# adaly/gridnext

Measured on AMD Instinct MI355X. Metric: spots/sec training throughput (multimodal f+g), higher is better.
Workload: dtype f32; 1 GPU; C4: multimodal f(DenseNet-121 @128px + count-MLP 2000 genes) + hex g on 78x64 Visium grids, 1 array (4992 spots) per GPU per step, f frozen/eval (tutorial mode), g trained with Adam, masked CE; spots_per_array=4992, parallelism=dp1

## Files before the change

### gridnext_amd/csrc/conv3x3.hip

```cpp
#include "fwd_common.h"

namespace {

constexpr int C3_BM = 128, C3_BN = 32;

__global__ __launch_bounds__(256) void conv3x3_kernel(const float* __restrict__ A, long lda,
                                                      const float* __restrict__ Wr, float* __restrict__ out, long ldc,
                                                      long M, int N, int K, int S, const float* __restrict__ scale,
                                                      const float* __restrict__ shift, int vecA, int vecW) {
    extern __shared__ __attribute__((aligned(16))) float lds[];
    const int strip = C3_BM + 2 * S + 2;
    float* As = lds;
    float* Bs = lds + strip * LDK;
    const int t = threadIdx.x, lane = t & 63, wave = t >> 6, h = lane >> 5, i = lane & 31;
    const long P0 = (long)blockIdx.x * C3_BM;
    const long base = P0 - S - 1;
    const int n0 = blockIdx.y * C3_BN;
    const bool has_act = scale != nullptr;

    const long P = P0 + 32 * wave + i;
    unsigned mask = 0;
    if (P < M) {
        const int rem = (int)(P % ((long)S * S));
        const int y = rem / S, x = rem - y * S;
#pragma unroll
        for (int tap = 0; tap < 9; ++tap) {
            const int yy = y + tap / 3 - 1, xx = x + tap % 3 - 1;
            if (yy >= 0 && yy < S && xx >= 0 && xx < S) mask |= 1u << tap;
        }
    }
    f32x16 acc;
#pragma unroll
    for (int r = 0; r < 16; ++r) acc[r] = 0.f;

    const int kq = t & 7;
    for (int k0 = 0; k0 < K; k0 += 32) {
        const int k = k0 + 4 * kq;
        const int valid = K - k;
        float4 sc4 = make_float4(1.f, 1.f, 1.f, 1.f), sh4 = make_float4(0.f, 0.f, 0.f, 0.f);
        if (has_act && valid > 0) {
            sc4 = ld4_safe(scale + k, valid, vecA);
            sh4 = ld4_safe(shift + k, valid, vecA);
        }
        __syncthreads();
        for (int row = t >> 3; row < strip; row += 32) {
            const long Pr = base + row;
            float4 v = make_float4(0.f, 0.f, 0.f, 0.f);
            if (Pr >= 0 && Pr < M && valid > 0) {
                v = ld4_safe(A + Pr * lda + k, valid, vecA);
                if (has_act) v = act4(v, sc4, sh4);
                if (valid < 4) {
                    if (valid < 2) v.y = 0.f;
                    if (valid < 3) v.z = 0.f;
                    v.w = 0.f;
                }
            }
            *reinterpret_cast<float4*>(&As[row * LDK + 4 * kq]) = v;
        }
        for (int idx = t >> 3; idx < 9 * 32; idx += 32) {
            const int tap = idx >> 5, n = n0 + (idx & 31);
            float4 v = make_float4(0.f, 0.f, 0.f, 0.f);
            if (n < N && valid > 0) v = ld4_safe(Wr + ((long)tap * N + n) * K + k, valid, vecW);
            *reinterpret_cast<float4*>(&Bs[idx * LDK + 4 * kq]) = v;
        }
        __syncthreads();
#pragma unroll
        for (int tap = 0; tap < 9; ++tap) {
            const int off = (S + 1) + (tap / 3 - 1) * S + (tap % 3 - 1);
            const bool ok = (mask >> tap) & 1u;
            const float* ap = &As[(32 * wave + i + off) * LDK + 4 * h];
            const float* bp = &Bs[(tap * 32 + i) * LDK + 4 * h];
#pragma unroll
            for (int s = 0; s < 4; ++s) {
                float4 a = ld4(ap + 8 * s);
                const float4 b = ld4(bp + 8 * s);
                if (!ok) a = make_float4(0.f, 0.f, 0.f, 0.f);
                acc = __builtin_amdgcn_mfma_f32_32x32x2f32(a.x, b.x, acc, 0, 0, 0);
                acc = __builtin_amdgcn_mfma_f32_32x32x2f32(a.y, b.y, acc, 0, 0, 0);
                acc = __builtin_amdgcn_mfma_f32_32x32x2f32(a.z, b.z, acc, 0, 0, 0);
                acc = __builtin_amdgcn_mfma_f32_32x32x2f32(a.w, b.w, acc, 0, 0, 0);
            }
        }
    }
    const int col = n0 + i;
    if (col < N) {
#pragma unroll
        for (int r = 0; r < 16; ++r) {
            const long row = P0 + 32 * wave + (r & 3) + 8 * (r >> 2) + 4 * h;
            if (row < M) out[row * ldc + col] = acc[r];
        }
    }
}

template <int NJ>
__global__ __launch_bounds__(256) void conv3x3_pipe_kernel(const float* __restrict__ A, long lda,
                                                           const float* __restrict__ Wr, float* __restrict__ out,
                                                           long ldc, long M, int N, int K, int S,
                                                           const float* __restrict__ scale,
                                                           const float* __restrict__ shift, int vecA, int vecW) {
    extern __shared__ __attribute__((aligned(16))) float lds[];
    const int strip = C3_BM + 2 * S + 2;
    float* As = lds;
    float* Bs = lds + strip * LDK;
    const int t = threadIdx.x, lane = t & 63, wave = t >> 6, h = lane >> 5, i = lane & 31;
    const long P0 = (long)blockIdx.x * C3_BM;
    const long base = P0 - S - 1;
    const int n0 = blockIdx.y * C3_BN;
    const bool has_act = scale != nullptr;
    const int kq = t & 7, r0 = t >> 3;

    const long P = P0 + 32 * wave + i;
    unsigned mask = 0;
    if (P < M) {
        const int rem = (int)(P % ((long)S * S));
        const int y = rem / S, x = rem - y * S;
#pragma unroll
        for (int tap = 0; tap < 9; ++tap) {
            const int yy = y + tap / 3 - 1, xx = x + tap % 3 - 1;
            if (yy >= 0 && yy < S && xx >= 0 && xx < S) mask |= 1u << tap;
        }
    }
    f32x16 acc0, acc1;
#pragma unroll
    for (int r = 0; r < 16; ++r) { acc0[r] = 0.f; acc1[r] = 0.f; }
    float* Zs = Bs + 9 * 32 * LDK;
    if (t < LDK) Zs[t] = 0.f;
    int aoff[9];
#pragma unroll
    for (int tap = 0; tap < 9; ++tap) {
        const int off = (S + 1) + (tap / 3 - 1) * S + (tap % 3 - 1);
        aoff[tap] = ((mask >> tap) & 1u) ? (32 * wave + i + off) * LDK + 4 * h : (strip + 9 * 32) * LDK;
    }

    float4 ra[NJ], rb[9], sc4, sh4;
    const int nload = n0 + r0 < N ? n0 + r0 : N - 1;
    auto fetch = [&](int k0) {
        const int k = k0 + 4 * kq;
        const int kc = k < K ? k : 0;
        sc4 = make_float4(1.f, 1.f, 1.f, 1.f);
        sh4 = make_float4(0.f, 0.f, 0.f, 0.f);
        if (has_act) {
            sc4 = ld4(scale + kc);
            sh4 = ld4(shift + kc);
        }
#pragma unroll
        for (int j = 0; j < NJ; ++j) {
            long Pr = base + r0 + 32 * j;
            Pr = Pr < 0 ? 0 : (Pr >= M ? M - 1 : Pr);
            ra[j] = ld4(A + Pr * lda + kc);
        }
#pragma unroll
        for (int j = 0; j < 9; ++j) rb[j] = ld4(Wr + ((long)j * N + nload) * K + kc);
    };
    const bool interior = base >= 0 && base + strip <= M && (K & 31) == 0 && n0 + C3_BN <= N;
    auto stash = [&](int k0) {
        if (interior) {
#pragma unroll
            for (int j = 0; j < NJ; ++j) {
                const int row = r0 + 32 * j;
                if (row >= strip) continue;
                float4 v = ra[j];
                if (has_act) v = act4(v, sc4, sh4);
                *reinterpret_cast<float4*>(&As[row * LDK + 4 * kq]) = v;
            }
#pragma unroll
            for (int j = 0; j < 9; ++j) *reinterpret_cast<float4*>(&Bs[(r0 + 32 * j) * LDK + 4 * kq]) = rb[j];
            return;
        }
        const bool kok = k0 + 4 * kq < K;
        const bool nok = n0 + r0 < N;
#pragma unroll
        for (int j = 0; j < NJ; ++j) {
            const int row = r0 + 32 * j;
            if (row >= strip) continue;
            const long Pr = base + row;
            float4 v = ra[j];
            if (has_act) v = act4(v, sc4, sh4);
            if (!(kok && Pr >= 0 && Pr < M)) v = make_float4(0.f, 0.f, 0.f, 0.f);
            *reinterpret_cast<float4*>(&As[row * LDK + 4 * kq]) = v;
        }
#pragma unroll
        for (int j = 0; j < 9; ++j) {
            float4 v = rb[j];
            if (!(kok && nok)) v = make_float4(0.f, 0.f, 0.f, 0.f);
            *reinterpret_cast<float4*>(&Bs[(r0 + 32 * j) * LDK + 4 * kq]) = v;
        }
    };

    const float* bbase = &Bs[i * LDK + 4 * h];
    fetch(0);
    __syncthreads();
    stash(0);
    __syncthreads();
    for (int k0 = 0; k0 < K; k0 += 32) {
        __builtin_amdgcn_s_setprio(3);
        if (k0 + 32 < K) fetch(k0 + 32);
        __builtin_amdgcn_s_setprio(0);
        float4 a = ld4(lds + aoff[0]), b = ld4(bbase);
#pragma unroll
        for (int step = 0; step < 36; ++step) {
            const int tap = step >> 2, sidx = step & 3;
            float4 na = a, nb = b;
            if (step < 35) {
                const int ntap = (step + 1) >> 2, ns = (step + 1) & 3;
                na = ld4(lds + aoff[ntap] + 8 * ns);
                nb = ld4(bbase + ntap * 32 * LDK + 8 * ns);
            }
            (void)tap; (void)sidx;
            acc0 = __builtin_amdgcn_mfma_f32_32x32x2f32(a.x, b.x, acc0, 0, 0, 0);
            acc1 = __builtin_amdgcn_mfma_f32_32x32x2f32(a.y, b.y, acc1, 0, 0, 0);
            acc0 = __builtin_amdgcn_mfma_f32_32x32x2f32(a.z, b.z, acc0, 0, 0, 0);
            acc1 = __builtin_amdgcn_mfma_f32_32x32x2f32(a.w, b.w, acc1, 0, 0, 0);
            a = na; b = nb;
            __builtin_amdgcn_sched_group_barrier(0x100, 2, 0);
            __builtin_amdgcn_sched_group_barrier(0x008, 4, 0);
        }
        if (k0 + 32 < K) {
            __builtin_amdgcn_s_setprio(3);
            __syncthreads();
            stash(k0 + 32);
            __syncthreads();
            __builtin_amdgcn_s_setprio(0);
        }
    }
    __builtin_amdgcn_s_setprio(3);
    const int col = n0 + i;
    if (col < N) {
#pragma unroll
        for (int r = 0; r < 16; ++r) {
            const long row = P0 + 32 * wave + (r & 3) + 8 * (r >> 2) + 4 * h;
            if (row < M) out[row * ldc + col] = acc0[r] + acc1[r];
        }
    }
}

#ifndef GNX_DMA_DBG
#define GNX_DMA_DBG 0
#endif

struct C3BnAdj {
    const float* a; int lda;
    const float* sc; const float* sh; const float* mean; const float* inv;
    float* slab;
};
template <int S, int NW, int KC, bool NK1 = false, bool H16 = false, bool O16 = false, bool BNADJ = false>
__global__ __launch_bounds__(64 * NW) void conv3x3_dma_kernel(const float* __restrict__ A, int lda,
                                                              const float* __restrict__ Wr, float* __restrict__ out,
                                                              int ldc, int M, int K, int N, C3BnAdj bn = C3BnAdj()) {
    constexpr int BM = 32 * NW;
    constexpr int strip = BM + 2 * S + 2;
    constexpr int SR = (strip + 15) & ~15;
    constexpr int ROWB = KC * 4;
    constexpr int GB = 16 * ROWB, PPG = GB / 1024;
    constexpr int BUFB = (SR + 9 * 32) * ROWB;
    constexpr int NPA = (SR >> 4) * PPG, NPW = 18 * PPG;
    constexpr int NSA = (NPA + NW - 1) / NW, NSW = (NPW + NW - 1) / NW;
    constexpr int SPT = KC / 8, STEPS = 9 * SPT;
    constexpr int ZB = 2 * BUFB;
    static_assert(NSA + NSW <= STEPS, "one DMA slot per MFMA step");
    static_assert(ZB + 2048 <= 160 * 1024, "LDS");
    __shared__ __attribute__((aligned(16))) char lds[ZB + 2048];
    const int t = threadIdx.x, lane = t & 63, h = lane >> 5, i = lane & 31;
    const int wave = __builtin_amdgcn_readfirstlane(t >> 6);
    for (int z = t; z < 512; z += 64 * NW) reinterpret_cast<float*>(lds + ZB)[z] = 0.f;
    const int T = M / BM;
    const int nk2 = NK1 ? N / 64 : K / (2 * KC);
    int G = gridDim.x;
    asm volatile("" : "+s"(G));
#ifndef GNX_XCD_ORDER
#define GNX_XCD_ORDER 1
#endif
    const int bx = blockIdx.x;
#if GNX_XCD_ORDER == 2
    const int bid = (G & 31) == 0 ? ((bx >> 5) << 5) + ((bx & 7) << 2) + ((bx >> 3) & 3) : bx;
#else
    const int bid = (GNX_XCD_ORDER && (G & 7) == 0) ? (bx & 7) * (G >> 3) + (bx >> 3) : bx;
#endif
    auto tile_of = [&](int round) {
        const int base = round * G;
        return base + (base + G <= T ? bid : bx);
    };
    const unsigned lb = lds_addr(lds);

    const unsigned voffA = ((unsigned)(lane & 15) * lda + 4 * (lane >> 4)) * 4u;
    const unsigned voffW = ((unsigned)(lane & 15) * K + 4 * (lane >> 4)) * 4u;
    int nround = 0, ntile = tile_of(0), nchunk = 0;
    const __amdgpu_buffer_rsrc_t rW = __builtin_amdgcn_make_buffer_rsrc(const_cast<float*>(Wr), 0, 9 * N * K * 4, 0x00020000);
    auto issue_slot = [&](auto slot_c, char* dst) {
        constexpr int slot = decltype(slot_c)::value;
        if constexpr (slot < NSA) {
            const int p = wave + NW * slot;
            if ((NPA % NW) && slot == NSA - 1 && p >= NPA) return;
            const int grp = p / PPG, part = p % PPG;
            const int row0 = ntile * BM - S - 1 + 16 * grp;
            char* d = dst + grp * GB + part * 1024;
            if (__builtin_expect(row0 >= 0 && row0 + 15 < M, 1)) {
                const __amdgpu_buffer_rsrc_t rs = __builtin_amdgcn_make_buffer_rsrc(
                    const_cast<float*>(A + (long)row0 * lda), 0, (15 * lda + K) * 4, 0x00020000);
                dma16_buf(rs, voffA, ((NK1 ? 0 : KC * nchunk) + 16 * part) * 4, lds_addr(d));
            } else {
                int Pr = row0 + (lane & 15);
                Pr = Pr < 0 ? 0 : (Pr >= M ? M - 1 : Pr);
                dma16_global(A + (long)Pr * lda + (NK1 ? 0 : KC * nchunk) + 16 * part + 4 * (lane >> 4), lds_addr(d));
            }
        } else {
            const int p = wave + NW * (slot - NSA);
            if ((NPW % NW) && slot == NSA + NSW - 1 && p >= NPW) return;
            if (H16 && !NK1 && nk2 == 1 && nround > 0) return;
            const int grp = p / PPG, part = p % PPG;
            dma16_buf(rW, voffW,
                      (((grp >> 1) * N + (NK1 ? 32 * nchunk : 0) + (grp & 1) * 16) * K + (NK1 ? 0 : KC * nchunk) + 16 * part) * 4,
                      lds_addr(dst + SR * ROWB + grp * GB + part * 1024));
        }
    };
    auto advance_next = [&]() {
        if (++nchunk == 2 * nk2) { nchunk = 0; ntile = tile_of(++nround); }
        if (ntile >= T) ntile = bid;
    };
    static_for<0, NSA + NSW>([&](auto sc) { issue_slot(sc, lds); });
    advance_next();

    const int R0 = 32 * wave + i + (S + 1);
    unsigned relA[9];
#pragma unroll
    for (int tap = 0; tap < 9; ++tap) {
        const int R = R0 + (tap / 3 - 1) * S + (tap % 3 - 1);
        relA[tap] = (R >> 4) * GB + (R & 15) * 16 + h * 256;
    }
    const unsigned relB = SR * ROWB + (i >> 4) * GB + (i & 15) * 16 + h * 256;
    const unsigned bB0 = lb + relB, bB1 = lb + BUFB + relB;

    bool stored = false;
    float adj_b[4] = {0.f, 0.f, 0.f, 0.f}, adj_g[4] = {0.f, 0.f, 0.f, 0.f};
    for (int round = 0, tile = tile_of(0); tile < T; tile = tile_of(++round)) {
        const int P = tile * BM + 32 * wave + i;
        const int rem = P % (S * S);
        const int y = rem / S, x = rem - y * S;
        unsigned bA0[9], bA1[9];
#pragma unroll
        for (int tap = 0; tap < 9; ++tap) {
            const int yy = y + tap / 3 - 1, xx = x + tap % 3 - 1;
            const bool ok = yy >= 0 && yy < S && xx >= 0 && xx < S;
            bA0[tap] = ok ? lb + relA[tap] : lb + ZB;
            bA1[tap] = ok ? lb + BUFB + relA[tap] : lb + ZB;
        }
        f32x16 acc0, acc1;
#pragma unroll
        for (int r = 0; r < 16; ++r) { acc0[r] = 0.f; acc1[r] = 0.f; }

        auto store16 = [&](int col0, auto ct_c) {
            if constexpr (BNADJ) {
                constexpr int ctc = decltype(ct_c)::value;
                const int col = col0 + i;
                const __amdgpu_buffer_rsrc_t ro = __builtin_amdgcn_make_buffer_rsrc(out + (long)tile * BM * ldc, 0, BM * ldc * 4,
                                                                                    0x00020000);
                const __amdgpu_buffer_rsrc_t ra = __builtin_amdgcn_make_buffer_rsrc(
                    const_cast<float*>(bn.a + (long)tile * BM * bn.lda), 0, BM * bn.lda * 4, 0x00020000);
                const int vo = ((32 * wave + 4 * h) * ldc + col) * 4, va = ((32 * wave + 4 * h) * bn.lda + col) * 4;
                float av[16];
#pragma unroll
                for (int r = 0; r < 16; ++r)
                    av[r] = __uint_as_float(__builtin_amdgcn_raw_buffer_load_b32(ra, va, ((r & 3) + 8 * (r >> 2)) * bn.lda * 4, 0));
                const float sc = bn.sc[col], sh = bn.sh[col], mu = bn.mean[col], is = bn.inv[col];
                const float rsc = 1.f / sc;
                float sb = adj_b[ctc], sg = adj_g[ctc];
#pragma unroll
                for (int r = 0; r < 16; ++r) {
                    const float d = av[r] > 0.f ? acc0[r] + acc1[r] : 0.f;
                    sb += d;
                    sg = fmaf(d, ((av[r] - sh) * rsc - mu) * is, sg);
                    __builtin_amdgcn_raw_buffer_store_b32(__float_as_uint(sc * d), ro, vo, ((r & 3) + 8 * (r >> 2)) * ldc * 4, 0);
                }
                adj_b[ctc] = sb;
                adj_g[ctc] = sg;
                stored = true;
                return;
            }
            if constexpr (O16) {
                _Float16* o16 = reinterpret_cast<_Float16*>(out);
                const __amdgpu_buffer_rsrc_t ro = __builtin_amdgcn_make_buffer_rsrc(o16 + (long)tile * BM * ldc, 0,
                                                                                    BM * ldc * 2, 0x00020000);
                const int vo = ((32 * wave + 4 * h) * ldc + col0 + i) * 2;
#pragma unroll
                for (int r = 0; r < 16; ++r) {
                    const _Float16 hv = (_Float16)(acc0[r] + acc1[r]);
                    __builtin_amdgcn_raw_buffer_store_b16(__builtin_bit_cast(short, hv), ro, vo,
                                                          ((r & 3) + 8 * (r >> 2)) * ldc * 2, 0);
                }
                stored = true;
                return;
            }
            const __amdgpu_buffer_rsrc_t ro = __builtin_amdgcn_make_buffer_rsrc(out + (long)tile * BM * ldc, 0, BM * ldc * 4,
                                                                                0x00020000);
            const int vo = ((32 * wave + 4 * h) * ldc + col0 + i) * 4;
#pragma unroll
            for (int r = 0; r < 16; ++r)
                __builtin_amdgcn_raw_buffer_store_b32(__float_as_uint(acc0[r] + acc1[r]), ro, vo,
                                                      ((r & 3) + 8 * (r >> 2)) * ldc * 4, 0);
            stored = true;
        };
        auto do_chunk = [&](auto par_c, int ct, auto ct_c) {
            constexpr int par = decltype(par_c)::value;
            if constexpr (NK1) {
#pragma unroll
                for (int r = 0; r < 16; ++r) { acc0[r] = 0.f; acc1[r] = 0.f; }
            }
            if (stored) asm volatile("s_waitcnt vmcnt(16)" ::: "memory");
            else asm volatile("s_waitcnt vmcnt(0)" ::: "memory");
            stored = false;
#if GNX_DMA_DBG != 2
            asm volatile("s_barrier" ::: "memory");
#endif
            char* nxt = lds + (par ? 0 : BUFB);
            const unsigned bB = par ? bB1 : bB0;
            auto rdA = [&](auto e_c) {
                constexpr int e = decltype(e_c)::value;
                return lds_read4<(e % SPT) * 512>(par ? bA1[e / SPT] : bA0[e / SPT]);
            };
            auto rdB = [&](auto e_c) {
                constexpr int e = decltype(e_c)::value;
                return lds_read4<(e / SPT) * 2 * GB + (e % SPT) * 512>(bB);
            };
            f32x4 a = rdA(std::integral_constant<int, 0>{}), bq = rdB(std::integral_constant<int, 0>{});
            static_for<0, STEPS>([&](auto step_c) {
                constexpr int step = decltype(step_c)::value;
                f32x4 na, nb;
                if constexpr (step < STEPS - 1) {
                    na = rdA(std::integral_constant<int, step + 1>{});
                    nb = rdB(std::integral_constant<int, step + 1>{});
                    asm volatile("s_waitcnt lgkmcnt(2)" : "+v"(a), "+v"(bq));
                } else {
                    asm volatile("s_waitcnt lgkmcnt(0)" : "+v"(a), "+v"(bq));
                }
                if constexpr (H16) {
                    typedef _Float16 half8 __attribute__((ext_vector_type(8)));
                    const half8 ah = __builtin_bit_cast(half8, a), bh = __builtin_bit_cast(half8, bq);
                    if constexpr (step & 1) acc1 = __builtin_amdgcn_mfma_f32_32x32x16_f16(ah, bh, acc1, 0, 0, 0);
                    else acc0 = __builtin_amdgcn_mfma_f32_32x32x16_f16(ah, bh, acc0, 0, 0, 0);
                } else {
                    acc0 = __builtin_amdgcn_mfma_f32_32x32x2f32(a[0], bq[0], acc0, 0, 0, 0);
                    acc1 = __builtin_amdgcn_mfma_f32_32x32x2f32(a[1], bq[1], acc1, 0, 0, 0);
                    acc0 = __builtin_amdgcn_mfma_f32_32x32x2f32(a[2], bq[2], acc0, 0, 0, 0);
                    acc1 = __builtin_amdgcn_mfma_f32_32x32x2f32(a[3], bq[3], acc1, 0, 0, 0);
                }
#if GNX_DMA_DBG != 1
                if constexpr (step < NSA + NSW) issue_slot(step_c, nxt);
#endif
                if constexpr (step < STEPS - 1) { a = na; bq = nb; }
            });
            advance_next();
            if constexpr (NK1) store16(32 * ct, ct_c);
        };
        if constexpr (BNADJ) {
            do_chunk(std::integral_constant<int, 0>{}, 0, std::integral_constant<int, 0>{});
            do_chunk(std::integral_constant<int, 1>{}, 1, std::integral_constant<int, 1>{});
            do_chunk(std::integral_constant<int, 0>{}, 2, std::integral_constant<int, 2>{});
            do_chunk(std::integral_constant<int, 1>{}, 3, std::integral_constant<int, 3>{});
        } else {
            for (int c2 = 0; c2 < nk2; ++c2) {
                do_chunk(std::integral_constant<int, 0>{}, 2 * c2, std::integral_constant<int, 0>{});
                do_chunk(std::integral_constant<int, 1>{}, 2 * c2 + 1, std::integral_constant<int, 0>{});
            }
        }
        if constexpr (!NK1) store16(0, std::integral_constant<int, 0>{});
    }
    asm volatile("s_waitcnt vmcnt(0)" ::: "memory");
    if constexpr (BNADJ) {
#pragma unroll
        for (int ct = 0; ct < 4; ++ct) {
            const float sb = adj_b[ct] + __shfl_xor(adj_b[ct], 32), sg = adj_g[ct] + __shfl_xor(adj_g[ct], 32);
            if (h == 0) {
                float* sl = bn.slab + (long)(blockIdx.x * NW + wave) * 2 * N + 32 * ct + i;
                sl[0] = sb;
                sl[N] = sg;
            }
        }
    }
}

constexpr int C3_ADJ_LANES = 16;
__global__ __launch_bounds__(64 * C3_ADJ_LANES) void c3_adj_reduce_kernel(const float* __restrict__ slab, int nblk, int C,
                                                                          float* __restrict__ dbeta,
                                                                          float* __restrict__ dgamma, int accumulate) {
    __shared__ float part[C3_ADJ_LANES][64];
    const int cl = threadIdx.x & 63, rl = threadIdx.x >> 6;
    const int idx = blockIdx.x * 64 + cl;
    float s0 = 0.f;
    if (idx < 2 * C) {
        const int q = idx / C, c = idx - q * C;
        const int per = (nblk + C3_ADJ_LANES - 1) / C3_ADJ_LANES;
        int b = rl * per;
        const int be = b + per < nblk ? b + per : nblk;
        for (; b + 16 <= be; b += 16) {
            float v[16];
#pragma unroll
            for (int u = 0; u < 16; ++u) v[u] = slab[((long)(b + u) * 2 + q) * C + c];
#pragma unroll
            for (int u = 0; u < 16; ++u) s0 += v[u];
        }
        for (; b < be; ++b) s0 += slab[((long)b * 2 + q) * C + c];
    }
    part[rl][cl] = s0;
    __syncthreads();
    if (rl == 0 && idx < 2 * C) {
        const int q = idx / C, c = idx - q * C;
        float tot = 0.f;
#pragma unroll
        for (int u = 0; u < C3_ADJ_LANES; ++u) tot += part[u][cl];
        float* dst = q == 0 ? dbeta : dgamma;
        if (dst) dst[c] = accumulate ? dst[c] + tot : tot;
    }
}

#ifndef GNX_WINO_DBG
#define GNX_WINO_DBG 0
#endif
template <int S>
__global__ __launch_bounds__(256) void conv3x3_wino_kernel(const float* __restrict__ A, int lda,
                                                          const float* __restrict__ Wu, float* __restrict__ out,
                                                          int ldc, int M, int K) {
    constexpr int BM = 256, NPAIR = 128;
    constexpr int RAWN = BM + 2 * S + 2, SRAW = (RAWN + 15) & ~15;
    constexpr int NV = NPAIR + S, NVR = (NV + 15) & ~15;
    constexpr int RAWB = SRAW * 64, UB = 12 * 32 * 64, VB = NVR * 64;
    constexpr int OFF_RAW = 0, OFF_U = 2 * RAWB, OFF_V = OFF_U + 2 * UB, OFF_Z = OFF_V + 4 * VB;
    static_assert(OFF_Z + 1024 <= 160 * 1024, "LDS");
    constexpr int NPR = SRAW / 16, NPU = 24;
    constexpr int NSR = (NPR + 3) / 4, NSU = NPU / 4;
    static_assert(NSR + NSU <= 24, "one DMA slot per MFMA step");
    __shared__ __attribute__((aligned(16))) char lds[OFF_Z + 1024];
    const int t = threadIdx.x, lane = t & 63, h = lane >> 5, i = lane & 31;
    const int wave = __builtin_amdgcn_readfirstlane(t >> 6);
    for (int z = t; z < 256; z += 256) reinterpret_cast<float*>(lds + OFF_Z)[z] = 0.f;
    const int T = (M + BM - 1) / BM;
    const int nk2 = K >> 5;
    int G = gridDim.x;
    asm volatile("" : "+s"(G));
    const int bx = blockIdx.x;
    const int bid = (G & 7) == 0 ? (bx & 7) * (G >> 3) + (bx >> 3) : bx;
    auto tile_of = [&](int round) {
        const int base = round * G;
        return base + (base + G <= T ? bid : bx);
    };
    const unsigned lb = lds_addr(lds);

    const int pix = ((lane & 15) - (wave & 1)) & 15;
    const unsigned voffA = ((unsigned)pix * lda + 4 * (lane >> 4)) * 4u;
    const unsigned voffU = ((unsigned)(lane & 15) * K + 4 * (lane >> 4)) * 4u;
    int nround = 0, ntile = tile_of(0), nchunk = 0;
    const __amdgpu_buffer_rsrc_t rU = __builtin_amdgcn_make_buffer_rsrc(const_cast<float*>(Wu), 0, 12 * 32 * K * 4, 0x00020000);
    auto issue_slot = [&](auto slot_c, int buf) {
        constexpr int slot = decltype(slot_c)::value;
        if constexpr (slot < NSR) {
            const int p = wave + 4 * slot;
            if ((NPR % 4) && slot == NSR - 1 && p >= NPR) return;
            const int row0 = ntile * BM - S - 1 + 16 * p;
            char* d = lds + OFF_RAW + buf * RAWB + p * 1024;
            if (__builtin_expect(row0 >= 0 && row0 + 15 < M, 1)) {
                const __amdgpu_buffer_rsrc_t rs = __builtin_amdgcn_make_buffer_rsrc(
                    const_cast<float*>(A + (long)row0 * lda), 0, (15 * lda + K) * 4, 0x00020000);
                dma16_buf(rs, voffA, 64 * nchunk, lds_addr(d));
            } else {
                int Pr = row0 + pix;
                Pr = Pr < 0 ? 0 : (Pr >= M ? M - 1 : Pr);
                dma16_global(A + (long)Pr * lda + 16 * nchunk + 4 * (lane >> 4), lds_addr(d));
            }
        } else {
            const int p = wave + 4 * (slot - NSR);
            dma16_buf(rU, voffU, (16 * p * K + 16 * nchunk) * 4, lds_addr(lds + OFF_U + buf * UB + p * 1024));
        }
    };
    auto advance_next = [&]() {
        if (++nchunk == 2 * nk2) { nchunk = 0; ntile = tile_of(++nround); }
        if (ntile >= T) ntile = bid;
    };
    static_for<0, NSR + NSU>([&](auto sc) { issue_slot(sc, 0); });
    advance_next();

    constexpr int NIT = (NVR * 4 + 255) / 256;
    const int r = 32 * wave + i;
    const unsigned fU = lb + OFF_U + (i >> 4) * 1024 + (i & 15) * 16 + h * 256;

    bool stored = false;
    for (int round = 0, tile = tile_of(0); tile < T; tile = tile_of(++round)) {
        const int P = tile * BM + 2 * r;
        const int y = (P % (S * S)) / S;
        unsigned bV[12];
#pragma unroll
        for (int dy = 0; dy < 3; ++dy) {
            const int jp = r + S / 2 + (dy - 1) * (S / 2);
            const bool ok = (dy == 1) || (dy == 0 ? y > 0 : y < S - 1);
#pragma unroll
            for (int xi = 0; xi < 4; ++xi)
                bV[dy * 4 + xi] = ok ? lb + OFF_V + xi * VB + (jp >> 4) * 1024 + (jp & 15) * 16 + h * 256 : lb + OFF_Z;
        }
        f32x16 acc[4][2];
#pragma unroll
        for (int xi = 0; xi < 4; ++xi)
#pragma unroll
            for (int q = 0; q < 2; ++q)
#pragma unroll
                for (int e = 0; e < 16; ++e) acc[xi][q][e] = 0.f;

        auto do_chunk = [&](auto par_c) {
            constexpr int par = decltype(par_c)::value;
            if (stored) asm volatile("s_waitcnt vmcnt(32)" ::: "memory");
            else asm volatile("s_waitcnt vmcnt(0)" ::: "memory");
            stored = false;
            asm volatile("s_barrier" ::: "memory");
#if GNX_WINO_DBG != 1
            {
                const char* raw = lds + OFF_RAW + par * RAWB;
#pragma unroll
                for (int j = 0; j < NIT; ++j) {
                    const int it = t + 256 * j;
                    const int c = it / NVR, jp = it - c * NVR;
                    if (it < NVR * 4 && jp < NV) {
                        const int xin = (2 * jp) & (S - 1);
                        auto at = [&](int q) {
                            return raw + (q >> 4) * 1024 + c * 256 + (((q & 15) + ((q >> 4) & 1)) & 15) * 16;
                        };
                        const char* zr = lds + OFF_Z;
                        typedef float f2 __attribute__((ext_vector_type(2)));
                        struct F4 { f2 lo, hi; };
                        auto rd = [&](const char* p) { return *reinterpret_cast<const F4*>(p); };
                        const F4 d0 = rd(xin == 0 ? zr : at(2 * jp)), d1 = rd(at(2 * jp + 1)), d2 = rd(at(2 * jp + 2)),
                                 d3 = rd(xin + 2 == S ? zr : at(2 * jp + 3));
                        char* v = lds + OFF_V + (jp >> 4) * 1024 + c * 256 + (jp & 15) * 16;
                        *reinterpret_cast<F4*>(v) = F4{d0.lo - d2.lo, d0.hi - d2.hi};
                        *reinterpret_cast<F4*>(v + VB) = F4{d1.lo + d2.lo, d1.hi + d2.hi};
                        *reinterpret_cast<F4*>(v + 2 * VB) = F4{d2.lo - d1.lo, d2.hi - d1.hi};
                        *reinterpret_cast<F4*>(v + 3 * VB) = F4{d1.lo - d3.lo, d1.hi - d3.hi};
                    }
                }
            }
#endif
            asm volatile("s_waitcnt lgkmcnt(0)" ::: "memory");
            asm volatile("s_barrier" ::: "memory");
            const unsigned bU = fU + par * UB;
            auto rdA = [&](auto e_c) {
                constexpr int e = decltype(e_c)::value;
                return lds_read4<(e & 1) * 512>(bV[e >> 1]);
            };
            auto rdB = [&](auto e_c) {
                constexpr int e = decltype(e_c)::value;
                return lds_read4<(e >> 1) * 2048 + (e & 1) * 512>(bU);
            };
            f32x4 a = rdA(std::integral_constant<int, 0>{}), bq = rdB(std::integral_constant<int, 0>{});
            static_for<0, 24>([&](auto step_c) {
                constexpr int step = decltype(step_c)::value;
                constexpr int xi = (step >> 1) & 3;
                f32x4 na, nb;
                if constexpr (step < 23) {
                    na = rdA(std::integral_constant<int, step + 1>{});
                    nb = rdB(std::integral_constant<int, step + 1>{});
                    asm volatile("s_waitcnt lgkmcnt(2)" : "+v"(a), "+v"(bq));
                } else {
                    asm volatile("s_waitcnt lgkmcnt(0)" : "+v"(a), "+v"(bq));
                }
                acc[xi][0] = __builtin_amdgcn_mfma_f32_32x32x2f32(a[0], bq[0], acc[xi][0], 0, 0, 0);
                acc[xi][1] = __builtin_amdgcn_mfma_f32_32x32x2f32(a[1], bq[1], acc[xi][1], 0, 0, 0);
                acc[xi][0] = __builtin_amdgcn_mfma_f32_32x32x2f32(a[2], bq[2], acc[xi][0], 0, 0, 0);
                acc[xi][1] = __builtin_amdgcn_mfma_f32_32x32x2f32(a[3], bq[3], acc[xi][1], 0, 0, 0);
#if GNX_WINO_DBG != 2
                if constexpr (step < NSR + NSU) issue_slot(step_c, par ^ 1);
#endif
                if constexpr (step < 23) { a = na; bq = nb; }
            });
            advance_next();
        };
        for (int c2 = 0; c2 < nk2; ++c2) {
            do_chunk(std::integral_constant<int, 0>{});
            do_chunk(std::integral_constant<int, 1>{});
        }
        {
            const int left = M - tile * BM;
            const __amdgpu_buffer_rsrc_t ro = __builtin_amdgcn_make_buffer_rsrc(
                out + (long)tile * BM * ldc, 0, (left < BM ? left : BM) * ldc * 4, 0x00020000);
            const int vo = (2 * (32 * wave + 4 * h) * ldc + i) * 4;
#pragma unroll
            for (int e = 0; e < 16; ++e) {
                const float m0 = acc[0][0][e] + acc[0][1][e], m1 = acc[1][0][e] + acc[1][1][e];
                const float m2 = acc[2][0][e] + acc[2][1][e], m3 = acc[3][0][e] + acc[3][1][e];
                const int row = 2 * ((e & 3) + 8 * (e >> 2));
                __builtin_amdgcn_raw_buffer_store_b32(__float_as_uint((m0 + m1) + m2), ro, vo, row * ldc * 4, 0);
                __builtin_amdgcn_raw_buffer_store_b32(__float_as_uint((m1 - m2) - m3), ro, vo, (row + 1) * ldc * 4, 0);
            }
        }
        stored = true;
    }
    asm volatile("s_waitcnt vmcnt(0)" ::: "memory");
}

__global__ void winograd_weights_kernel(const float* __restrict__ w, float* __restrict__ wu, int N, int K) {
    const long idx = (long)blockIdx.x * blockDim.x + threadIdx.x;
    const long total = (long)3 * N * K;
    if (idx >= total) return;
    const int k = (int)(idx % K), n = (int)((idx / K) % N), dy = (int)(idx / ((long)K * N));
    const float* g = w + ((long)n * K + k) * 9 + dy * 3;
    const float g0 = g[0], g1 = g[1], g2 = g[2];
    const long nk = (long)N * K;
    float* u = wu + (long)dy * 4 * nk + (long)n * K + k;
    u[0] = g0;
    u[nk] = 0.5f * ((g0 + g2) + g1);
    u[2 * nk] = 0.5f * ((g0 + g2) - g1);
    u[3 * nk] = g2;
}

__global__ void repack3x3_kernel(const float* __restrict__ w, float* __restrict__ wr, int N, int K) {
    const long idx = (long)blockIdx.x * blockDim.x + threadIdx.x;
    const long total = (long)9 * N * K;
    if (idx >= total) return;
    const int k = (int)(idx % K), n = (int)((idx / K) % N), tap = (int)(idx / ((long)K * N));
    wr[idx] = w[((long)n * K + k) * 9 + tap];
}

struct C3Plan { int rc, form, wgs, wgy; };
enum { GNX_C3_GENERIC = 0, GNX_C3_PIPE5 = 1, GNX_C3_PIPE6 = 2, GNX_C3_PIPE7 = 3, GNX_C3_PIPE9 = 4, GNX_C3_DMA4 = 5, GNX_C3_DMA8 = 6,
       GNX_C3_DMAG4 = 7, GNX_C3_DMAG8 = 8, GNX_C3_WINO = 9 };

bool c3_dma_s(int S) {
    return S == 4 || S == 7 || S == 8 || S == 14 || S == 16 || S == 28 || S == 32 || S == 56 || S == 64;
}
bool c3_pow2_s(int S) { return S == 4 || S == 8 || S == 16 || S == 32 || S == 64; }
bool c3_eight_waves(long M, int S) { return S <= 32 && M % 256 == 0 && M / 256 >= 1024; }
int c3_persistent_wgs(long M, int bm) { return (int)(M / bm > 256 ? 256 : M / bm); }

size_t c3_lds_bytes(int S) { return ((size_t)(C3_BM + 2 * S + 2) * LDK + 9 * 32 * LDK + LDK) * sizeof(float); }

C3Plan conv3x3_plan(const float* A, long lda, const float* Wr, const float* out, long ldc, long M, int N, int K, int S,
                    const float* scale, const float* shift) {
    C3Plan p = {GNX_OK, GNX_C3_GENERIC, 0, 0};
    if (!A || !Wr || !out || M < 0 || N <= 0 || K <= 0 || S <= 0 || lda < K || ldc < N || (!scale) != (!shift) ||
        (M % ((long)S * S)) != 0) {
        p.rc = GNX_ERR_BAD_ARG;
        return p;
    }
    if (M == 0) return p;
    if (c3_lds_bytes(S) > 160 * 1024) {
        p.rc = GNX_ERR_UNSUPPORTED;
        return p;
    }
    const bool vecA = al16(A) && lda % 4 == 0 && K % 4 == 0 && (!scale || (al16(scale) && al16(shift)));
    const bool vecW = al16(Wr) && K % 4 == 0;
    const bool fast = vecA && vecW;
    const bool dma = !scale && fast && (M % C3_BM) == 0 && M * (lda > ldc ? lda : ldc) < (1L << 31) && c3_dma_s(S);
    const bool wide = c3_eight_waves(M, S);
    if (dma && ((N == C3_BN && (K & 63) == 0) || (K == 32 && (N & 63) == 0))) {
        const bool dgrad = !(N == C3_BN && (K & 63) == 0);
        p.form = dgrad ? (wide ? GNX_C3_DMAG8 : GNX_C3_DMAG4) : (wide ? GNX_C3_DMA8 : GNX_C3_DMA4);
        p.wgs = c3_persistent_wgs(M, wide ? 256 : 128);
        p.wgy = 1;
        return p;
    }
    const int nj = (int)gnx_cdiv(C3_BM + 2 * S + 2, 32);
    p.form = !fast || nj > 9 ? GNX_C3_GENERIC : nj <= 5 ? GNX_C3_PIPE5 : nj == 6 ? GNX_C3_PIPE6 : nj == 7 ? GNX_C3_PIPE7
                                                                                                        : GNX_C3_PIPE9;
    p.wgs = (int)gnx_cdiv(M, C3_BM);
    p.wgy = (int)gnx_cdiv(N, C3_BN);
    return p;
}

C3Plan conv3x3_wino_plan(const float* A, long lda, const float* Wu, const float* out, long ldc, long M, int N, int K, int S) {
    C3Plan p = {GNX_OK, GNX_C3_WINO, 0, 1};
    if (!A || !Wu || !out || M < 0 || N <= 0 || K <= 0 || S <= 0 || lda < K || ldc < N || (M % ((long)S * S)) != 0)
        p.rc = GNX_ERR_BAD_ARG;
    else if (N != 32 || (K & 31) != 0 || !al16(A) || !al16(Wu) || lda % 4 != 0 || M * (lda > ldc ? lda : ldc) >= (1L << 31))
        p.rc = GNX_ERR_UNSUPPORTED;
    else if (M > 0) {
        if (c3_pow2_s(S)) p.wgs = c3_persistent_wgs(M + 255, 256);
        else p.rc = GNX_ERR_UNSUPPORTED;
    }
    return p;
}

C3Plan conv3x3_dgrad_bn_plan(const float* dY, long lddy, const float* Wb, const float* A_act, long lda, const float* dX,
                             long lddx, long M, int N, int K, int S, const float* scale, const float* shift, const float* mean,
                             const float* invstd, const float* workspace) {
    C3Plan p = {GNX_OK, 4, 0, 1};
    if (!dY || !Wb || !A_act || !dX || !scale || !shift || !mean || !invstd || !workspace || M < 0 || N <= 0 || K <= 0 ||
        S <= 0 || lddy < K || lda < N || lddx < N || (M % ((long)S * S)) != 0)
        p.rc = GNX_ERR_BAD_ARG;
    else if (K != 32 || N != 128 || (M % C3_BM) != 0 || !al16(dY) || !al16(Wb) || lddy % 4 != 0 ||
             M * (lddy > lddx ? (lddy > lda ? lddy : lda) : (lddx > lda ? lddx : lda)) >= (1L << 31))
        p.rc = GNX_ERR_UNSUPPORTED;
    else if (M > 0) {
        if (!c3_pow2_s(S)) {
            p.rc = GNX_ERR_UNSUPPORTED;
            return p;
        }
        p.form = c3_eight_waves(M, S) ? 8 : 4;
        p.wgs = c3_persistent_wgs(M, 32 * p.form);
    }
    return p;
}

C3Plan conv3x3_f16_plan(const void* A16, long lda16, const void* Wr16, const void* out, long ldc, long M, int N, int K, int S) {
    C3Plan p = {GNX_OK, 4, 0, 1};
    if (!A16 || !Wr16 || !out || M < 0 || N <= 0 || K <= 0 || S <= 0 || lda16 < K || ldc < N || (M % ((long)S * S)) != 0)
        p.rc = GNX_ERR_BAD_ARG;
    else if (N != C3_BN || (K & 127) != 0 || (M % C3_BM) != 0 || (lda16 & 7) != 0 || !al16(A16) || !al16(Wr16) ||
             M * (lda16 > ldc ? lda16 : ldc) >= (1L << 31))
        p.rc = GNX_ERR_UNSUPPORTED;
    else if (M > 0) {
        if (!c3_pow2_s(S)) {
            p.rc = GNX_ERR_UNSUPPORTED;
            return p;
        }
        p.form = c3_eight_waves(M, S) ? 8 : 4;
        p.wgs = c3_persistent_wgs(M, 32 * p.form);
    }
    return p;
}

int c3_answer(const C3Plan& p, int* workgroups) {
    if (workgroups) *workgroups = p.rc == GNX_OK ? p.wgs : 0;
    return p.rc != GNX_OK ? p.rc : p.form;
}

}

GNX_EXPORT int gnx_conv3x3_form(const float* A, long lda, const float* Wr, const float* out, long ldc, long M, int N, int K,
                                int S, const float* scale, const float* shift, int* workgroups) {
    return c3_answer(conv3x3_plan(A, lda, Wr, out, ldc, M, N, K, S, scale, shift), workgroups);
}
GNX_EXPORT int gnx_conv3x3_winograd_form(const float* A, long lda, const float* Wu, const float* out, long ldc, long M, int N,
                                         int K, int S, int* workgroups) {
    return c3_answer(conv3x3_wino_plan(A, lda, Wu, out, ldc, M, N, K, S), workgroups);
}
GNX_EXPORT int gnx_conv3x3_dgrad_bnrelu_bwd_form(const float* dY, long lddy, const float* Wb, const float* A_act, long lda,
                                                 const float* dX, long lddx, long M, int N, int K, int S, const float* scale,
                                                 const float* shift, const float* mean, const float* invstd,
                                                 const float* workspace, int* workgroups) {
    return c3_answer(conv3x3_dgrad_bn_plan(dY, lddy, Wb, A_act, lda, dX, lddx, M, N, K, S, scale, shift, mean, invstd, workspace),
                     workgroups);
}
GNX_EXPORT int gnx_conv3x3_f16_dma_form(const void* A16, long lda16, const void* Wr16, const void* out, long ldc, long M, int N,
                                        int K, int S, int* workgroups) {
    return c3_answer(conv3x3_f16_plan(A16, lda16, Wr16, out, ldc, M, N, K, S), workgroups);
}

GNX_EXPORT int gnx_repack_conv3x3(const float* w, float* wr, int N, int K, hipStream_t stream) {
    if (!w || !wr || N <= 0 || K <= 0) return GNX_ERR_BAD_ARG;
    repack3x3_kernel<<<gnx_cdiv(9L * N * K, 256), 256, 0, stream>>>(w, wr, N, K);
    return gnx_launch_status();
}

GNX_EXPORT int gnx_winograd_conv3x3_weights(const float* w, float* wu, int N, int K, hipStream_t stream) {
    if (!w || !wu || N <= 0 || K <= 0) return GNX_ERR_BAD_ARG;
    winograd_weights_kernel<<<gnx_cdiv(3L * N * K, 256), 256, 0, stream>>>(w, wu, N, K);
    return gnx_launch_status();
}

GNX_EXPORT int gnx_conv3x3_winograd(const float* A, long lda, const float* Wu, float* out, long ldc, long M, int N, int K,
                                    int S, hipStream_t stream) {
    const C3Plan p = conv3x3_wino_plan(A, lda, Wu, out, ldc, M, N, K, S);
    if (p.rc != GNX_OK || p.wgs == 0) return p.rc;
#define GNX_WINO(SS)                                                                                        \
    conv3x3_wino_kernel<SS><<<p.wgs, 256, 0, stream>>>(A, (int)lda, Wu, out, (int)ldc, (int)M, K);           \
    return gnx_launch_status()
    switch (S) {
        case 4: GNX_WINO(4);
        case 8: GNX_WINO(8);
        case 16: GNX_WINO(16);
        case 32: GNX_WINO(32);
        case 64: GNX_WINO(64);
        default: return GNX_ERR_UNSUPPORTED;
    }
#undef GNX_WINO
}

GNX_EXPORT long gnx_conv3x3_dgrad_bn_workspace(long M, int N) { return 256L * 8 * 2 * N; }

GNX_EXPORT int gnx_conv3x3_dgrad_bnrelu_bwd(const float* dY, long lddy, const float* Wb, const float* A_act, long lda,
                                            float* dX, long lddx, long M, int N, int K, int S, const float* scale,
                                            const float* shift, const float* mean, const float* invstd, float* dgamma,
                                            float* dbeta, int accumulate, float* workspace, hipStream_t stream) {
    const C3Plan p = conv3x3_dgrad_bn_plan(dY, lddy, Wb, A_act, lda, dX, lddx, M, N, K, S, scale, shift, mean, invstd, workspace);
    if (p.rc != GNX_OK || p.wgs == 0) return p.rc;
    C3BnAdj bn = {A_act, (int)lda, scale, shift, mean, invstd, workspace};
    const int nblk = p.wgs * p.form;
#define GNX_DMAA(SS)                                                                                              \
    do {                                                                                                          \
        if constexpr (SS <= 32) {                                                                                 \
            if (p.form == 8) {                                                                                    \
                conv3x3_dma_kernel<SS, 8, 32, true, false, false, true><<<p.wgs, 512, 0, stream>>>(               \
                    dY, (int)lddy, Wb, dX, (int)lddx, (int)M, K, N, bn);                                          \
                break;                                                                                            \
            }                                                                                                     \
        }                                                                                                         \
        conv3x3_dma_kernel<SS, 4, 32, true, false, false, true><<<p.wgs, 256, 0, stream>>>(                       \
            dY, (int)lddy, Wb, dX, (int)lddx, (int)M, K, N, bn);                                                  \
    } while (0)
    switch (S) {
        case 4: GNX_DMAA(4); break;
        case 8: GNX_DMAA(8); break;
        case 16: GNX_DMAA(16); break;
        case 32: GNX_DMAA(32); break;
        case 64: GNX_DMAA(64); break;
        default: return GNX_ERR_UNSUPPORTED;
    }
#undef GNX_DMAA
    if (dgamma || dbeta)
        c3_adj_reduce_kernel<<<gnx_cdiv(2 * N, 64), 64 * C3_ADJ_LANES, 0, stream>>>(workspace, nblk, N, dbeta, dgamma, accumulate);
    return gnx_launch_status();
}

GNX_EXPORT int gnx_conv3x3_bnrelu(const float* A, long lda, const float* Wr, float* out, long ldc, long M, int N, int K,
                                  int S, const float* scale, const float* shift, hipStream_t stream) {
    const C3Plan p = conv3x3_plan(A, lda, Wr, out, ldc, M, N, K, S, scale, shift);
    if (p.rc != GNX_OK || p.wgs == 0) return p.rc;
    const size_t lds_bytes = c3_lds_bytes(S);
    static size_t configured = 0;
    if (lds_bytes > configured) {
        if (hipFuncSetAttribute(reinterpret_cast<const void*>(conv3x3_kernel), hipFuncAttributeMaxDynamicSharedMemorySize,
                                (int)lds_bytes) != hipSuccess)
            return GNX_ERR_LAUNCH;
        configured = lds_bytes;
    }
    const int vecA = al16(A) && lda % 4 == 0 && K % 4 == 0 && (!scale || (al16(scale) && al16(shift)));
    const int vecW = al16(Wr) && K % 4 == 0;
    const dim3 grid(p.wgs, p.wgy);
#define GNX_PIPE(NJ)                                                                                              \
    do {                                                                                                          \
        static size_t conf = 0;                                                                                   \
        if (lds_bytes > conf) {                                                                                   \
            if (hipFuncSetAttribute(reinterpret_cast<const void*>(conv3x3_pipe_kernel<NJ>),                       \
                                    hipFuncAttributeMaxDynamicSharedMemorySize, (int)lds_bytes) != hipSuccess)    \
                return GNX_ERR_LAUNCH;                                                                            \
            conf = lds_bytes;                                                                                     \
        }                                                                                                         \
        conv3x3_pipe_kernel<NJ><<<grid, 256, lds_bytes, stream>>>(A, lda, Wr, out, ldc, M, N, K, S, scale, shift, \
                                                                  vecA, vecW);                                    \
    } while (0)
#define GNX_DMA(SS, NK1)                                                                                         \
    do {                                                                                                         \
        if constexpr (SS <= 32) {                                                                                \
            if (eight) {                                                                                         \
                conv3x3_dma_kernel<SS, 8, 32, NK1><<<p.wgs, 512, 0, stream>>>(A, (int)lda, Wr, out, (int)ldc,    \
                                                                              (int)M, K, N);                     \
                return gnx_launch_status();                                                                      \
            }                                                                                                    \
        }                                                                                                        \
        conv3x3_dma_kernel<SS, 4, 32, NK1><<<p.wgs, 256, 0, stream>>>(A, (int)lda, Wr, out, (int)ldc, (int)M, K, \
                                                                      N);                                        \
        return gnx_launch_status();                                                                              \
    } while (0)
#define GNX_DMA_S(NK1)                                                                                           \
    switch (S) {                                                                                                 \
        case 4: GNX_DMA(4, NK1);                                                                                 \
        case 7: GNX_DMA(7, NK1);                                                                                 \
        case 8: GNX_DMA(8, NK1);                                                                                 \
        case 14: GNX_DMA(14, NK1);                                                                               \
        case 16: GNX_DMA(16, NK1);                                                                               \
        case 28: GNX_DMA(28, NK1);                                                                               \
        case 32: GNX_DMA(32, NK1);                                                                               \
        case 56: GNX_DMA(56, NK1);                                                                               \
        case 64: GNX_DMA(64, NK1);                                                                               \
        default: return GNX_ERR_UNSUPPORTED;                      \
    }
    const bool eight = p.form == GNX_C3_DMA8 || p.form == GNX_C3_DMAG8;
    switch (p.form) {
        case GNX_C3_DMA4:
        case GNX_C3_DMA8: GNX_DMA_S(false);
        case GNX_C3_DMAG4:
        case GNX_C3_DMAG8: GNX_DMA_S(true);
        case GNX_C3_PIPE5: GNX_PIPE(5); break;
        case GNX_C3_PIPE6: GNX_PIPE(6); break;
        case GNX_C3_PIPE7: GNX_PIPE(7); break;
        case GNX_C3_PIPE9: GNX_PIPE(9); break;
        default: conv3x3_kernel<<<grid, 256, lds_bytes, stream>>>(A, lda, Wr, out, ldc, M, N, K, S, scale, shift, vecA, vecW);
    }
#undef GNX_DMA_S
#undef GNX_DMA
#undef GNX_PIPE
    return gnx_launch_status();
}

template <bool O16>
static int conv3x3_f16_dma_launch(const void* A16, long lda16, const void* Wr16, float* out, long ldc, long M, int N, int K,
                                  int S, hipStream_t stream) {
    const C3Plan p = conv3x3_f16_plan(A16, lda16, Wr16, out, ldc, M, N, K, S);
    if (p.rc != GNX_OK || p.wgs == 0) return p.rc;
    const float* A = reinterpret_cast<const float*>(A16);
    const float* Wr = reinterpret_cast<const float*>(Wr16);
    const int Kf = K / 2, ldaf = (int)(lda16 / 2);
#define GNX_DMAH(SS)                                                                                             \
    do {                                                                                                         \
        if constexpr (SS <= 32) {                                                                                \
            if (p.form == 8) {                                                                                   \
                conv3x3_dma_kernel<SS, 8, 32, false, true, O16><<<p.wgs, 512, 0, stream>>>(A, ldaf, Wr, out,     \
                                                                                         (int)ldc, (int)M, Kf, N); \
                return gnx_launch_status();                                                                      \
            }                                                                                                    \
        }                                                                                                        \
        conv3x3_dma_kernel<SS, 4, 32, false, true, O16><<<p.wgs, 256, 0, stream>>>(A, ldaf, Wr, out, (int)ldc,   \
                                                                                 (int)M, Kf, N);                 \
        return gnx_launch_status();                                                                              \
    } while (0)
    switch (S) {
        case 4: GNX_DMAH(4);
        case 8: GNX_DMAH(8);
        case 16: GNX_DMAH(16);
        case 32: GNX_DMAH(32);
        case 64: GNX_DMAH(64);
        default: break;
    }
#undef GNX_DMAH
    return GNX_ERR_UNSUPPORTED;
}

GNX_EXPORT int gnx_conv3x3_f16_dma(const void* A16, long lda16, const void* Wr16, float* out, long ldc, long M, int N, int K,
                                   int S, hipStream_t stream) {
    return conv3x3_f16_dma_launch<false>(A16, lda16, Wr16, out, ldc, M, N, K, S, stream);
}
GNX_EXPORT int gnx_conv3x3_f16_dma_h(const void* A16, long lda16, const void* Wr16, void* out16, long ldc16, long M, int N,
                                     int K, int S, hipStream_t stream) {
    return conv3x3_f16_dma_launch<true>(A16, lda16, Wr16, reinterpret_cast<float*>(out16), ldc16, M, N, K, S, stream);
}
```

Before: 86520 spots/s.

## Load Winograd input tiles into registers and transform directly into double-buffered LDS

The Winograd 3x3 conv kernel no longer DMAs a raw input strip into LDS and then re-reads it to build the V transform. Each thread now issues buffer loads straight into registers, interleaved with the MFMA steps, and applies the input transform when writing V into a double-buffered LDS region. This drops the raw staging buffer and one barrier round per chunk, so the next chunk's V can be prepared while the current chunk computes. In exchange it uses more VGPRs, relies on buffer out-of-range handling for zero padding (with a shifted base for tile 0), and adds an lda limit to the plan.

```diff
diff --git a/gridnext_amd/csrc/conv3x3.hip b/gridnext_amd/csrc/conv3x3.hip
--- a/gridnext_amd/csrc/conv3x3.hip
+++ b/gridnext_amd/csrc/conv3x3.hip
@@ -515,23 +515,28 @@
 #ifndef GNX_WINO_DBG
 #define GNX_WINO_DBG 0
 #endif
+constexpr long C3_WINO_MAX_LDA = 1L << 21;
 template <int S>
 __global__ __launch_bounds__(256) void conv3x3_wino_kernel(const float* __restrict__ A, int lda,
                                                           const float* __restrict__ Wu, float* __restrict__ out,
                                                           int ldc, int M, int K) {
     constexpr int BM = 256, NPAIR = 128;
-    constexpr int RAWN = BM + 2 * S + 2, SRAW = (RAWN + 15) & ~15;
     constexpr int NV = NPAIR + S, NVR = (NV + 15) & ~15;
-    constexpr int RAWB = SRAW * 64, UB = 12 * 32 * 64, VB = NVR * 64;
-    constexpr int OFF_RAW = 0, OFF_U = 2 * RAWB, OFF_V = OFF_U + 2 * UB, OFF_Z = OFF_V + 4 * VB;
-    static_assert(OFF_Z + 1024 <= 160 * 1024, "LDS");
-    constexpr int NPR = SRAW / 16, NPU = 24;
-    constexpr int NSR = (NPR + 3) / 4, NSU = NPU / 4;
-    static_assert(NSR + NSU <= 24, "one DMA slot per MFMA step");
-    __shared__ __attribute__((aligned(16))) char lds[OFF_Z + 1024];
+    constexpr int UB = 12 * 32 * 64, VB = NVR * 64;
+    constexpr int VD = 4 * VB + 1024;
+    constexpr int OFF_U = 0, OFF_V = 2 * UB, OFF_Z = OFF_V + 4 * VB, LDSB = OFF_V + 2 * VD;
+    static_assert(LDSB <= 160 * 1024, "LDS");
+    static_assert(VD + 512 < 65536 && 3 * VB < 65536, "ds immediate offsets");
+    constexpr int NSU = 24 / 4;
+    constexpr int NIT = (NVR / 16 + 3) / 4, NSL = 2 * NIT;
+    static_assert(NIT == 3 && NSL + NSU <= 24 && NVR / 16 > 4 * (NIT - 1), "item layout");
+    constexpr int ROWS = 2 * NVR + 2;
+    constexpr unsigned VOOR = 0xFFFFFF00u;
+    __shared__ __attribute__((aligned(16))) char lds[LDSB];
     const int t = threadIdx.x, lane = t & 63, h = lane >> 5, i = lane & 31;
     const int wave = __builtin_amdgcn_readfirstlane(t >> 6);
-    for (int z = t; z < 256; z += 256) reinterpret_cast<float*>(lds + OFF_Z)[z] = 0.f;
+    reinterpret_cast<float*>(lds + OFF_Z)[t] = 0.f;
+    reinterpret_cast<float*>(lds + OFF_Z + VD)[t] = 0.f;
     const int T = (M + BM - 1) / BM;
     const int nk2 = K >> 5;
     int G = gridDim.x;
@@ -544,44 +549,95 @@
     };
     const unsigned lb = lds_addr(lds);
 
-    const int pix = ((lane & 15) - (wave & 1)) & 15;
-    const unsigned voffA = ((unsigned)pix * lda + 4 * (lane >> 4)) * 4u;
+    unsigned voff[NIT][4];
+    auto set_voff = [&](int shift) {
+#pragma unroll
+        for (int j = 0; j < NIT; ++j) {
+            const int c = lane >> 4, jp = 16 * (wave + 4 * j) + (lane & 15);
+            const bool live = jp < NV;
+            const int xin = (2 * jp) & (S - 1);
+#pragma unroll
+            for (int e = 0; e < 4; ++e) {
+                const bool zero = !live || (e == 0 && xin == 0) || (e == 3 && xin + 2 == S);
+                voff[j][e] = zero ? VOOR : (unsigned)((2 * jp + e - shift) * lda + 4 * c) * 4u;
+            }
+        }
+    };
     const unsigned voffU = ((unsigned)(lane & 15) * K + 4 * (lane >> 4)) * 4u;
-    int nround = 0, ntile = tile_of(0), nchunk = 0;
+    int nround = 0, ntile = tile_of(0), nchunk = 0, nshift = ntile == 0 ? S + 1 : 0;
+    set_voff(nshift);
     const __amdgpu_buffer_rsrc_t rU = __builtin_amdgcn_make_buffer_rsrc(const_cast<float*>(Wu), 0, 12 * 32 * K * 4, 0x00020000);
-    auto issue_slot = [&](auto slot_c, int buf) {
-        constexpr int slot = decltype(slot_c)::value;
-        if constexpr (slot < NSR) {
-            const int p = wave + 4 * slot;
-            if ((NPR % 4) && slot == NSR - 1 && p >= NPR) return;
-            const int row0 = ntile * BM - S - 1 + 16 * p;
-            char* d = lds + OFF_RAW + buf * RAWB + p * 1024;
-            if (__builtin_expect(row0 >= 0 && row0 + 15 < M, 1)) {
-                const __amdgpu_buffer_rsrc_t rs = __builtin_amdgcn_make_buffer_rsrc(
-                    const_cast<float*>(A + (long)row0 * lda), 0, (15 * lda + K) * 4, 0x00020000);
-                dma16_buf(rs, voffA, 64 * nchunk, lds_addr(d));
-            } else {
-                int Pr = row0 + pix;
-                Pr = Pr < 0 ? 0 : (Pr >= M ? M - 1 : Pr);
-                dma16_global(A + (long)Pr * lda + 16 * nchunk + 4 * (lane >> 4), lds_addr(d));
-            }
-        } else {
-            const int p = wave + 4 * (slot - NSR);
-            dma16_buf(rU, voffU, (16 * p * K + 16 * nchunk) * 4, lds_addr(lds + OFF_U + buf * UB + p * 1024));
-        }
+    auto raw_rsrc = [&]() {
+        const int rb = ntile * BM - S - 1 + nshift;
+        const int left = M - rb;
+        const unsigned nrows = left < ROWS ? left : ROWS;
+        return __builtin_amdgcn_make_buffer_rsrc(const_cast<float*>(A + (long)rb * lda + 16 * nchunk), 0,
+                                                 (int)(((nrows - 1) * (unsigned)lda + 16) * 4u), 0x00020000);
+    };
+    auto issue_u = [&](int slot, int buf) {
+        const int p = wave + 4 * slot;
+        dma16_buf(rU, voffU, (16 * p * K + 16 * nchunk) * 4, lds_addr(lds + OFF_U + buf * UB + p * 1024));
     };
     auto advance_next = [&]() {
-        if (++nchunk == 2 * nk2) { nchunk = 0; ntile = tile_of(++nround); }
-        if (ntile >= T) ntile = bid;
-    };
-    static_for<0, NSR + NSU>([&](auto sc) { issue_slot(sc, 0); });
-    advance_next();
-
-    constexpr int NIT = (NVR * 4 + 255) / 256;
+        if (++nchunk == 2 * nk2) {
+            nchunk = 0;
+            ntile = tile_of(++nround);
+            if (ntile >= T) ntile = bid;
+            const int sh = ntile == 0 ? S + 1 : 0;
+            if (sh != nshift) {
+                nshift = sh;
+                set_voff(sh);
+            }
+        }
+    };
+    unsigned wv[NIT];
+#pragma unroll
+    for (int j = 0; j < NIT; ++j) wv[j] = lb + OFF_V + (wave + 4 * j) * 1024 + (lane >> 4) * 256 + (lane & 15) * 16;
+    [[maybe_unused]] const bool last_item = wave + 4 * (NIT - 1) < NVR / 16;
+    auto wait_raw = [&](f32x4 (&d)[NIT][4]) {
+        asm volatile("s_waitcnt vmcnt(%12)"
+                     : "+v"(d[0][0]), "+v"(d[0][1]), "+v"(d[0][2]), "+v"(d[0][3]), "+v"(d[1][0]), "+v"(d[1][1]), "+v"(d[1][2]),
+                       "+v"(d[1][3]), "+v"(d[2][0]), "+v"(d[2][1]), "+v"(d[2][2]), "+v"(d[2][3])
+                     : "n"(NSU));
+    };
+    auto put_item = [&](f32x4 (&d)[NIT][4], int j, int buf) {
+#if GNX_WINO_DBG != 1
+        if (j < NIT - 1 || last_item) {
+            const unsigned v = wv[j] + buf * VD;
+            const f32x4 v0 = d[j][0] - d[j][2], v1 = d[j][1] + d[j][2], v2 = d[j][2] - d[j][1], v3 = d[j][1] - d[j][3];
+            asm volatile("ds_write_b128 %0, %1" ::"v"(v), "v"(v0) : "memory");
+            asm volatile("ds_write_b128 %0, %1 offset:%2" ::"v"(v), "v"(v1), "n"(VB) : "memory");
+            asm volatile("ds_write_b128 %0, %1 offset:%2" ::"v"(v), "v"(v2), "n"(2 * VB) : "memory");
+            asm volatile("ds_write_b128 %0, %1 offset:%2" ::"v"(v), "v"(v3), "n"(3 * VB) : "memory");
+        }
+#endif
+    };
+    auto publish = [&]() { asm volatile("s_waitcnt vmcnt(0) lgkmcnt(0)\n\ts_barrier" ::: "memory"); };
+    auto feed = [&](f32x4 (&d)[NIT][4], int buf) {
+        wait_raw(d);
+#pragma unroll
+        for (int j = 0; j < NIT; ++j) put_item(d, j, buf);
+        publish();
+    };
+    auto load_piece = [&](f32x4& d, unsigned vo, const __amdgpu_buffer_rsrc_t& rs) {
+        asm volatile("buffer_load_dwordx4 %0, %1, %2, 0 offen" : "=&v"(d) : "v"(vo), "s"(rs) : "memory");
+    };
+    {
+        const __amdgpu_buffer_rsrc_t rs = raw_rsrc();
+        f32x4 d[NIT][4];
+#pragma unroll
+        for (int j = 0; j < NIT; ++j)
+#pragma unroll
+            for (int e = 0; e < 4; ++e) load_piece(d[j][e], voff[j][e], rs);
+#pragma unroll
+        for (int s = 0; s < NSU; ++s) issue_u(s, 0);
+        advance_next();
+        feed(d, 0);
+    }
+
     const int r = 32 * wave + i;
     const unsigned fU = lb + OFF_U + (i >> 4) * 1024 + (i & 15) * 16 + h * 256;
 
-    bool stored = false;
     for (int round = 0, tile = tile_of(0); tile < T; tile = tile_of(++round)) {
         const int P = tile * BM + 2 * r;
         const int y = (P % (S * S)) / S;
@@ -604,43 +660,18 @@
 
         auto do_chunk = [&](auto par_c) {
             constexpr int par = decltype(par_c)::value;
-            if (stored) asm volatile("s_waitcnt vmcnt(32)" ::: "memory");
-            else asm volatile("s_waitcnt vmcnt(0)" ::: "memory");
-            stored = false;
-            asm volatile("s_barrier" ::: "memory");
-#if GNX_WINO_DBG != 1
-            {
-                const char* raw = lds + OFF_RAW + par * RAWB;
-#pragma unroll
-                for (int j = 0; j < NIT; ++j) {
-                    const int it = t + 256 * j;
-                    const int c = it / NVR, jp = it - c * NVR;
-                    if (it < NVR * 4 && jp < NV) {
-                        const int xin = (2 * jp) & (S - 1);
-                        auto at = [&](int q) {
-                            return raw + (q >> 4) * 1024 + c * 256 + (((q & 15) + ((q >> 4) & 1)) & 15) * 16;
-                        };
-                        const char* zr = lds + OFF_Z;
-                        typedef float f2 __attribute__((ext_vector_type(2)));
-                        struct F4 { f2 lo, hi; };
-                        auto rd = [&](const char* p) { return *reinterpret_cast<const F4*>(p); };
-                        const F4 d0 = rd(xin == 0 ? zr : at(2 * jp)), d1 = rd(at(2 * jp + 1)), d2 = rd(at(2 * jp + 2)),
-                                 d3 = rd(xin + 2 == S ? zr : at(2 * jp + 3));
-                        char* v = lds + OFF_V + (jp >> 4) * 1024 + c * 256 + (jp & 15) * 16;
-                        *reinterpret_cast<F4*>(v) = F4{d0.lo - d2.lo, d0.hi - d2.hi};
-                        *reinterpret_cast<F4*>(v + VB) = F4{d1.lo + d2.lo, d1.hi + d2.hi};
-                        *reinterpret_cast<F4*>(v + 2 * VB) = F4{d2.lo - d1.lo, d2.hi - d1.hi};
-                        *reinterpret_cast<F4*>(v + 3 * VB) = F4{d1.lo - d3.lo, d1.hi - d3.hi};
-                    }
-                }
-            }
+            [[maybe_unused]] const __amdgpu_buffer_rsrc_t rs = raw_rsrc();
+            f32x4 d[NIT][4];
+#if GNX_WINO_DBG == 2
+#pragma unroll
+            for (int j = 0; j < NIT; ++j)
+#pragma unroll
+                for (int e = 0; e < 4; ++e) d[j][e] = f32x4{0.f, 0.f, 0.f, 0.f};
 #endif
-            asm volatile("s_waitcnt lgkmcnt(0)" ::: "memory");
-            asm volatile("s_barrier" ::: "memory");
             const unsigned bU = fU + par * UB;
             auto rdA = [&](auto e_c) {
                 constexpr int e = decltype(e_c)::value;
-                return lds_read4<(e & 1) * 512>(bV[e >> 1]);
+                return lds_read4<(e & 1) * 512 + par * VD>(bV[e >> 1]);
             };
             auto rdB = [&](auto e_c) {
                 constexpr int e = decltype(e_c)::value;
@@ -663,11 +694,17 @@
                 acc[xi][0] = __builtin_amdgcn_mfma_f32_32x32x2f32(a[2], bq[2], acc[xi][0], 0, 0, 0);
                 acc[xi][1] = __builtin_amdgcn_mfma_f32_32x32x2f32(a[3], bq[3], acc[xi][1], 0, 0, 0);
 #if GNX_WINO_DBG != 2
-                if constexpr (step < NSR + NSU) issue_slot(step_c, par ^ 1);
+                if constexpr (step < NSL) {
+                    load_piece(d[step >> 1][2 * (step & 1)], voff[step >> 1][2 * (step & 1)], rs);
+                    load_piece(d[step >> 1][2 * (step & 1) + 1], voff[step >> 1][2 * (step & 1) + 1], rs);
+                } else if constexpr (step < NSL + NSU) {
+                    issue_u(step - NSL, par ^ 1);
+                }
 #endif
                 if constexpr (step < 23) { a = na; bq = nb; }
             });
             advance_next();
+            feed(d, par ^ 1);
         };
         for (int c2 = 0; c2 < nk2; ++c2) {
             do_chunk(std::integral_constant<int, 0>{});
@@ -687,7 +724,6 @@
                 __builtin_amdgcn_raw_buffer_store_b32(__float_as_uint((m1 - m2) - m3), ro, vo, (row + 1) * ldc * 4, 0);
             }
         }
-        stored = true;
     }
     asm volatile("s_waitcnt vmcnt(0)" ::: "memory");
 }
@@ -765,7 +801,8 @@
     C3Plan p = {GNX_OK, GNX_C3_WINO, 0, 1};
     if (!A || !Wu || !out || M < 0 || N <= 0 || K <= 0 || S <= 0 || lda < K || ldc < N || (M % ((long)S * S)) != 0)
         p.rc = GNX_ERR_BAD_ARG;
-    else if (N != 32 || (K & 31) != 0 || !al16(A) || !al16(Wu) || lda % 4 != 0 || M * (lda > ldc ? lda : ldc) >= (1L << 31))
+    else if (N != 32 || (K & 31) != 0 || !al16(A) || !al16(Wu) || lda % 4 != 0 || M * (lda > ldc ? lda : ldc) >= (1L << 31) ||
+             lda > C3_WINO_MAX_LDA)
         p.rc = GNX_ERR_UNSUPPORTED;
     else if (M > 0) {
         if (c3_pow2_s(S)) p.wgs = c3_persistent_wgs(M + 255, 256);
```

Result: no change. 86360 spots/s (median of 2 runs) (-0.2%).
